# HLLMR/stratum-dsp

Measured on AMD Instinct MI355X. Metric: tracks/sec full analyze_audio(), 3-min 44.1 kHz mono, at 1/2/4/8 MI355X, higher is better.
Workload: dtype f32

## Files before the change

### stratum-dsp_amd/csrc/k_features.hip

```cpp
#include <stdexcept>
#include <type_traits>

#include "kernels.hpp"

namespace sdsp {



typedef const __attribute__((address_space(4))) int* ConstI;
typedef const __attribute__((address_space(4))) MelChunk* ConstMC;

template <int CW, int W, int KK>
__global__ __launch_bounds__(FT_FRAMES) __attribute__((amdgpu_waves_per_eu(KK > 0 ? 3 : 1))) void k_features(const RowMap rm,
                                                        const uint64_t* __restrict__ frame_pfx,
                                                        const uint64_t* __restrict__ tile_pfx, int T, FeatParams P,
                                                        const MelPlan* __restrict__ mel, float* __restrict__ E,
                                                        float* __restrict__ H, float* __restrict__ SFX,
                                                        float* __restrict__ SFO, float* __restrict__ MEL,
                                                        uint64_t total) {
    static_assert((W & (W - 1)) == 0, "W must be a power of two");
    constexpr int ROWS = FT_FRAMES;
    constexpr int LS = W + 1;
    __shared__ float2 ML[ROWS][LS];
    __shared__ sd_logtab2_t ltab[512];
    __shared__ sd_ln2tab_t etab[129];
    static_assert(KK == 0 || CW + 2 * KK <= W, "window halo must fit the ring");
    for (int q = threadIdx.x; q < 512; q += FT_FRAMES) ltab[q] = SD_LOGTAB9_D[q];
    for (int q = threadIdx.x; q < 129; q += FT_FRAMES) etab[q] = sd_ln2tab_from(q);

    const uint64_t gb = blockIdx.x;
    const int trk = find_track(tile_pfx, T, gb);
    const int64_t F = (int64_t)(frame_pfx[trk + 1] - frame_pfx[trk]);
    const int64_t f0 = (int64_t)(gb - tile_pfx[trk]) * FT_STEP;
    const uint64_t g0 = frame_pfx[trk];
    const int i = threadIdx.x;
    const bool helper = (i & 63) == 0;
    const int ro = i;
    const int64_t f = f0 - 1 + 63 * (i >> 6) + (i & 63);
    const bool own_ok = f >= 0 && f < F;
    const bool valid = !helper && f < F;
    const bool has_prev = valid && f >= 1;
    const int K = KK > 0 ? KK : P.K, B = P.B;
    const uint64_t g = g0 + (uint64_t)f;

    float e[4] = {0, 0, 0, 0}, h[4] = {0, 0, 0, 0}, sx[4] = {0, 0, 0, 0}, so = 0.0f;
    float eb = 0.0f, hb = 0.0f, sb = 0.0f;
    int cur = 0;
    auto band_of = [&](int b) {
        int v = 0;
#pragma unroll
        for (int q = 3; q >= 1; q--)
            if (P.band_on[q] && b >= P.bs[q] && b < P.be[q]) v = q;
        return v;
    };
    auto flush = [&]() {
        if (cur == 1) e[1] = eb, h[1] = hb, sx[1] = sb;
        else if (cur == 2) e[2] = eb, h[2] = hb, sx[2] = sb;
        else if (cur == 3) e[3] = eb, h[3] = hb, sx[3] = sb;
        eb = hb = sb = 0.0f;
    };
    float accA = 0.0f, accB = 0.0f;
    int mA = 0;
    float* melA = MEL;
    const uint32_t mel_vo = valid ? (uint32_t)g * 4u : 0xFFFFFFF0u;
    auto mel_rsrc = [&]() {
        return __builtin_amdgcn_make_buffer_rsrc((void*)melA, (short)0, (int)(uint32_t)(total * 4u), 0x00020000);
    };
    const uint64_t ra0 = rm.rowA0[trk], rb0 = rm.rowB0 ? rm.rowB0[trk] : ra0 + (uint64_t)rm.offB;
    auto row_of = [&](int64_t fr, bool* odd) {
        *odd = fr & 1;
        return (*odd ? rb0 + (uint64_t)(fr >> 1) * (uint64_t)rm.stepB : ra0 + (uint64_t)(fr >> 1) * (uint64_t)rm.stepA);
    };
    auto fmax_of = [&](int64_t fr) {
        bool odd;
        const uint64_t r = row_of(fr, &odd);
        return odd ? rm.fmaxB[r] : rm.fmaxA[r];
    };
    const float mx_c = own_ok ? fmax_of(f) : 0.0f;
    const bool cn = mx_c > EPS;
    const float yr = cn ? 1.0f / mx_c : 0.0f;
    const bool q_frame_ok = !cn || mx_c <= 0x1p100f;
    const uint32_t q_lim = __float_as_uint(sd_maxf(0x1p-100f, mx_c * 0x1p-120f)) - 1u;
    uint32_t q_lo = 0xFFFFFFFFu, q_hi = 0u;
    auto quot = [&](float m) {
        const uint32_t u = __float_as_uint(m);
        q_lo = min(q_lo, u - 1u);
        q_hi = max(q_hi, u);
        const float q0 = m * yr;
        return __builtin_fmaf(__builtin_fmaf(-mx_c, q0, m), yr, q0);
    };
    auto quot_redo = [&](int c0, int nb, float so_start) {
        const bool miss = !q_frame_ok || q_lo < q_lim || q_hi >= 0x7F800000u;
        q_lo = 0xFFFFFFFFu;
        q_hi = 0u;
        if (__builtin_expect(__builtin_amdgcn_ballot_w64(miss) == 0, 1)) return;
        so = so_start;
        for (int j = 0; j < nb; j++) {
            const float m = ML[ro][(c0 + j) & (W - 1)].x;
            const float cv = cn ? m / mx_c : 0.0f;
            const float pv = __builtin_bit_cast(
                float, __builtin_amdgcn_update_dpp(0, __builtin_bit_cast(int, cv), 0x138, 0xf, 0xf, true));
            const float d = max_bnn(cv - pv, 0.0f);
            so += d * d;
        }
    };

    const int lane = i & 63, wrow = i & ~63;
    const int sub = lane / CW, jj = lane % CW;
    const int64_t fw = f0 - 1 + 63 * (i >> 6);

    constexpr int RSTEP = 64 / CW;
    constexpr int NLD = CW;
    const float* rowp[NLD];
#pragma unroll
    for (int u = 0; u < NLD; u++) {
        const int64_t fr = fw + sub + u * RSTEP;
        rowp[u] = rm.magsA;
        if (fr >= 0 && fr < F) {
            bool odd;
            const uint64_t row = row_of(fr, &odd);
            rowp[u] = (odd ? rm.magsB : rm.magsA) + row * (uint64_t)P.stride;
        }
    }
    float nx[NLD];
    uint32_t row_ok = 0;
#pragma unroll
    for (int u = 0; u < NLD; u++) {
        const int64_t fr = fw + sub + u * RSTEP;
        row_ok |= (uint32_t)(fr >= 0 && fr < F) << u;
    }
    auto load = [&](int b0) {
        const int b = b0 + jj;
// ... 32 lines not shown
        asm volatile("" ::: "memory");
        if (c0 + CW < B) load(c0 + CW + K);
        const int nb = B - c0 < CW ? B - c0 : CW;
        if (__builtin_amdgcn_ballot_w64(valid) == 0) continue;
        float Rw[KK > 0 ? CW + 2 * KK : 1];
        constexpr bool VHK = KK > 0 && 2 * KK == CW;
        float Wm[VHK ? CW : 1];
        const int rp = lane > 0 ? ro - 1 : ro;
        if (KK > 0) {
#pragma unroll
            for (int q = 0; q < (KK > 0 ? CW + 2 * KK : 1); q++) Rw[q] = ML[rp][(c0 - KK + q) & (W - 1)].y;
            if constexpr (VHK) {
                float suf[CW], pre[CW];
                suf[CW - 1] = Rw[CW - 1];
#pragma unroll
                for (int q = CW - 2; q >= 0; q--) suf[q] = max_bnn(Rw[q], suf[q + 1]);
                pre[0] = Rw[CW];
#pragma unroll
                for (int q = 1; q < CW; q++) pre[q] = max_bnn(pre[q - 1], Rw[CW + q]);
#pragma unroll
                for (int q = 0; q < CW; q++) Wm[q] = max_bnn(suf[q], pre[q]);
            }
        }
        if constexpr (VHK) {
            const int cf = ((ConstI)P.chunk_flags)[c0 / CW];
            if (cf & (FT_CHUNK_FAST | FT_CHUNK_MEL)) {
                const int vbc = cf & 3;
                if (vbc != cur) {
                    flush();
                    cur = vbc;
                }
                const float so_start = so;
                auto walk = [&](auto mel_tag, auto reg_tag, auto noband_tag) {
                    constexpr bool MEL = decltype(mel_tag)::value;
                    constexpr bool REG = decltype(reg_tag)::value;
                    constexpr bool NOBAND = decltype(noband_tag)::value;
                    MelChunk mc{};
                    const ConstMC mcp = (ConstMC)P.mel_chunks + c0 / CW;
                    if constexpr (MEL) {
                        mc.bits = mcp->bits;
#pragma unroll
                        for (int j = 0; j < CW; j++) mc.w0[j] = mcp->w0[j], mc.w1[j] = mcp->w1[j];
                    }
                    float bfv[CW];
#pragma unroll
                    for (int j = 0; j < CW; j++) bfv[j] = mcp->bf[j];
#pragma unroll
                    for (int j = 0; j < CW; j++) {
                        const int b = c0 + j;
                        const int s = b & (W - 1);
                        const float2 ml = ML[ro][s];
                        const float m = ml.x;
                        const float ee = m * m;
                        const float hh = bfv[j] * m * m;
                        e[0] += ee;
                        h[0] += hh;
                        const float lc = ml.y;
                        const float cv = quot(m);
                        const float pv = __builtin_bit_cast(
                            float, __builtin_amdgcn_update_dpp(0, __builtin_bit_cast(int, cv), 0x138, 0xf, 0xf, true));
                        const float d = max_bnn(cv - pv, 0.0f);
                        so += d * d;
                        const float df = max_bnn(lc - Wm[j], 0.0f);
                        const float df2 = df * df;
                        sx[0] += df2;
                        if (!NOBAND && vbc) {
                            eb += ee;
                            hb += hh;
                            sb += df2;
                        }
                        if constexpr (MEL) {
                            const uint32_t pb = mc.bits >> (4 * j);
                            for (uint32_t q = pb & 3; q > 0; q--) {
                                __builtin_amdgcn_raw_buffer_store_b32(__float_as_uint(accA), mel_rsrc(), mel_vo, 0, 0);
                                accA = accB;
                                accB = 0.0f;
                                mA++;
                                melA += total;
                            }
                            if constexpr (REG) {
                                if (__float_as_uint(mc.w0[j]) << 1) accA += lc * mc.w0[j];
                                if (__float_as_uint(mc.w1[j]) << 1) accB += lc * mc.w1[j];
                            } else if (mc.w0[j] != 0.0f) {
                                if (pb & 4) accB += lc * mc.w0[j];
                                else accA += lc * mc.w0[j];
                            }
                            if (!REG && mc.w1[j] != 0.0f) {
                                if (pb & 8) accB += lc * mc.w1[j];
                                else accA += lc * mc.w1[j];
                            }
                        }
                    }
                };
                if (cf & FT_CHUNK_MELREG)
                    walk(std::true_type{}, std::true_type{}, std::false_type{});
                else if (cf & FT_CHUNK_MEL)
                    walk(std::true_type{}, std::false_type{}, std::false_type{});
                else if (vbc == 0)
                    walk(std::false_type{}, std::false_type{}, std::true_type{});
                else
                    walk(std::false_type{}, std::false_type{}, std::false_type{});
                quot_redo(c0, CW, so_start);
                continue;
            }
        }
        const float so_start = so;
#pragma unroll
        for (int j = 0; j < CW; j++) {
            if (j >= nb) continue;
            const int b = c0 + j;
            const int s = b & (W - 1);
            const float2 ml = ML[ro][s];
            const float m = ml.x;
            const float ee = m * m;
            const float hh = (float)b * m * m;
            e[0] += ee;
            h[0] += hh;
            const int vb = band_of(b);
            if (vb != cur) {
                flush();
                cur = vb;
            }
            if (vb) {
                eb += ee;
                hb += hh;
            }
            const float lc = ml.y;
            const float cv = quot(m);
            const float pv = __builtin_bit_cast(
                float, __builtin_amdgcn_update_dpp(0, __builtin_bit_cast(int, cv), 0x138 , 0xf, 0xf, true));
            if (P.n_mels > 0) {
                const MelPlan mp = mel[b];
                for (int q = 0; q < mp.nflush; q++) {
                    if (valid) MEL[(uint64_t)mA * total + g] = accA;
                    accA = accB;
                    accB = 0.0f;
                    mA++;
                    melA += total;
                }
                if (mp.w0 != 0.0f) {
                    if (mp.s0 == 0) accA += lc * mp.w0;
                    else accB += lc * mp.w0;
                }
                if (mp.w1 != 0.0f) {
                    if (mp.s1 == 0) accA += lc * mp.w1;
                    else accB += lc * mp.w1;
                }
            }
            {
                const float d = max_bnn(cv - pv, 0.0f);
                so += d * d;
                const int lo = b - K < 0 ? 0 : b - K;
                const int hi = b + K + 1 < B ? b + K + 1 : B;
                float pm = 0.0f;
                if constexpr (KK > 0) {
                    if constexpr (VHK) {
                        pm = Wm[j];
                    } else {
                        pm = Rw[j];
#pragma unroll
                        for (int q = 1; q <= 2 * KK; q++) pm = max_bnn(pm, Rw[j + q]);
                    }
                } else {
                    for (int q = lo; q < hi; q++) pm = max_bnn(pm, ML[rp][q & (W - 1)].y);
                }
                const float df = max_bnn(lc - pm, 0.0f);
                const float df2 = df * df;
                sx[0] += df2;
                if (vb) {
                    const int bsv = P.bs[vb], bev = P.be[vb];
                    if (lo < bsv || hi > bev) {
                        const int lb = lo < bsv ? bsv : lo;
                        const int hbd = hi > bev ? bev : hi;
                        float pmb = 0.0f;
                        if constexpr (KK > 0) {
#pragma unroll
                            for (int q = 0; q <= 2 * KK; q++)
                                if (b - KK + q >= lb && b - KK + q < hbd) pmb = max_bnn(pmb, Rw[j + q]);
                        } else {
                            for (int q = lb; q < hbd; q++) pmb = max_bnn(pmb, ML[rp][q & (W - 1)].y);
                        }
                        const float db = max_bnn(lc - pmb, 0.0f);
                        sb += db * db;
                    } else {
                        sb += df2;
                    }
                }
            }
        }
        quot_redo(c0, nb, so_start);
    }
    flush();
    if (!valid) return;
    for (; mA < P.n_mels; mA++) {
        MEL[(uint64_t)mA * total + g] = accA;
        accA = accB;
        accB = 0.0f;
    }
#pragma unroll
    for (int v = 0; v < 4; v++) {
        E[(uint64_t)v * total + g] = e[v];
        H[(uint64_t)v * total + g] = h[v];
    }
    if (has_prev) {
        const uint64_t gp = g - 1;
        SFO[gp] = __builtin_sqrtf(so);
#pragma unroll
        for (int v = 0; v < 4; v++) SFX[(uint64_t)v * total + gp] = __builtin_sqrtf(sx[v]);
    }
}

void launch_features(const RowMap& mags, const uint64_t* frame_pfx, const uint64_t* tile_pfx,
                     int T, uint64_t n_tiles, const FeatParams& P, const MelPlan* mel, float* E, float* H, float* SFX,
                     float* SFO, float* MEL, uint64_t total, hipStream_t st) {
    if (n_tiles == 0) return;
    if (total >= (1ull << 30)) throw std::runtime_error("launch_features: too many frames for one launch");

    if (P.K == 4)
        hipLaunchKernelGGL((k_features<8, 16, 4>), dim3((unsigned)n_tiles), dim3(FT_FRAMES), 0, st, mags,
                           frame_pfx, tile_pfx, T, P, mel, E, H, SFX, SFO, MEL, total);
    else if (P.K <= 4)
        hipLaunchKernelGGL((k_features<8, 16, 0>), dim3((unsigned)n_tiles), dim3(FT_FRAMES), 0, st, mags,
                           frame_pfx, tile_pfx, T, P, mel, E, H, SFX, SFO, MEL, total);
    else
        hipLaunchKernelGGL((k_features<16, 32, 0>), dim3((unsigned)n_tiles), dim3(FT_FRAMES), 0, st, mags,
                           frame_pfx, tile_pfx, T, P, mel, E, H, SFX, SFO, MEL, total);
}

}
```

### stratum-dsp_amd/csrc/kernels.hpp

```cpp
#pragma once

#include <hip/hip_runtime.h>
#include <stdint.h>

#include "sdsp_device.hpp"

namespace sdsp {

constexpr int NVAR = 5;

struct MelChunk {
    uint32_t bits;
    float w0[8], w1[8];
    float bf[8];
};
struct FeatParams {
    int B;
    int stride;
    int K;
    int bs[4], be[4];
    int band_on[4];
    int n_mels;
    const int* chunk_flags;
    const MelChunk* mel_chunks;
};
constexpr int FT_CHUNK_FAST = 4, FT_CHUNK_MEL = 8, FT_CHUNK_MELREG = 16;
struct MelPlan {
    int nflush;
    int s0, s1;
    float w0, w1;
};
#ifndef SDSP_PK_CH
#define SDSP_PK_CH 16384
#endif
constexpr int PK_CH = SDSP_PK_CH;
constexpr int FT_FRAMES = 256;
constexpr int FT_STEP = FT_FRAMES - FT_FRAMES / 64;
struct RowMap {
    const float *magsA, *magsB, *fmaxA, *fmaxB;
    const uint64_t *rowA0, *rowB0;
    int offB, stepA, stepB;
};
constexpr int FT_KMAX = 8;
constexpr int FT_MELMAX = 48;

struct NovParams {
    float ws, we, wh, wsum;
    int lmw, smw;
    int band_on[4];
};

struct FftTgParams {
    int P;
    int b_lo, K;
    float fres;
    int lds;
};
struct SelParams {
    float min_bpm, max_bpm, ac_tol;
    float w[NVAR];
// ... 176 lines not shown
void launch_loudness_gain(const float* x, const uint64_t* in_off, const uint64_t* n_raw, const uint64_t* chunk_pfx,
                          int T, uint64_t n_chunks, unsigned int* chunk_bits, unsigned int* peak_bits,
                          const LoudnessParams& P, float* gain, int* status, hipStream_t st);
void launch_frame_rms(const float* x, const uint64_t* src_off, const float* gain, const uint64_t* n_len,
                      const uint64_t* frame_pfx, int T, uint64_t total, int fs, int hop, float* rms, hipStream_t st, bool per_frame_kernel = false);
void launch_trim(const float* rms, const uint64_t* frame_pfx, int T, const uint64_t* n_raw, int hop, float thr,
                 uint64_t min_frames, int enable, uint64_t* trim_start, uint64_t* trim_end, hipStream_t st,
                 const uint64_t* base_pfx = nullptr, int stride = 1);
void launch_frame_rms_from_raw(const float* raw, const uint64_t* raw_base, const float* x, const uint64_t* src_off,
                               const float* gain, const uint64_t* n_trim, const uint64_t* frame_pfx, int T, uint64_t total,
                               int fs, int hop, float* rms, hipStream_t st);
void launch_energy_onsets(const float* rms, const uint64_t* frame_pfx, const uint64_t* n_trim, int hop, float factor,
                          uint32_t* out, const uint64_t* out_off, int* out_n, int T, hipStream_t st);
void launch_flux_onsets(const float* sfo, const float* hfc, const float* hpe, float* scratch, const uint64_t* frame_pfx,
                        const uint64_t* n_trim, int hop, float pct, uint32_t* out, const uint64_t* out_off,
                        int* out_n, int T, hipStream_t st);
void launch_consensus(const uint32_t* energy, const uint64_t* e_off, const int* e_n, const uint32_t* flux_on,
                      const uint64_t* f_off, const int* f_n, uint64_t kind_stride, int T, uint32_t tol, int enable,
                      const int* has_mags, uint32_t* chosen, const uint64_t* c_off, int* c_n, uint32_t* scratch,
                      hipStream_t st, int hpss = 0);
void launch_features(const RowMap& mags, const uint64_t* frame_pfx, const uint64_t* tile_pfx,
                     int T, uint64_t n_tiles, const FeatParams& P, const MelPlan* mel, float* E, float* H, float* SFX,
                     float* SFO, float* MEL, uint64_t total, hipStream_t st);
void launch_novelty(const float* E, const float* H, const float* SFX, const uint64_t* frame_pfx, int T, uint64_t total,
                    const NovParams& P, float* scratch, float* nov, float* nov_sum, const float* MEL, int n_mels,
                    int mel_k, bool mel_on, unsigned int* mel_max, hipStream_t st);
void launch_fft_tempogram(const int* items, int n_items, int T, const float* nov, const float* nov_sum,
                          const uint64_t* frame_pfx, uint64_t total, const FftTgParams& P, const cx* tw, const cx* rt,
                          cx* gscratch, const uint64_t* out_off, float* out_bpm, float* out_pow, hipStream_t st);
void launch_acf_tempogram(const int* items, int n_items, const float* nov, const uint64_t* frame_pfx, uint64_t total,
                          const float* bpm_grid, const int* lag_grid, int NB, float* out_bpm, float* out_str,
                          hipStream_t st);
void launch_tempo_select(int n_items, const int* active, const float* fft_bpm, const float* fft_pow, const uint64_t* fft_off,
                         const int* fft_k, const float* acf_bpm, const float* acf_str, const uint64_t* acf_off,
                         const SelParams& P, TempoEst* est, float* cand, int cand_cap, hipStream_t st);
void launch_multires(const int* tracks, int n_items, const float* c256, const int* n256, const float* c512,
                     const int* n512, const float* c1024, const int* n1024, int cap256, int cap512, int cap1024,
                     const TempoEst* base_est, const float* nov512, const uint64_t* fpfx512, const MrParams& P,
                     TempoEst* mr_est, int* used, float* final_bpm, float* final_conf, hipStream_t st, MrDbg* dbg = nullptr);
void launch_beat(const int* tracks, int n_items, const uint32_t* onsets, const uint64_t* on_off, const int* on_n,
                 uint32_t sr, const float* bpm, const float* conf, float* scratch, const uint64_t* beat_off,
                 const int* beat_cap, float* beats, float* downs, BeatOut* out, hipStream_t st);
void launch_beat_compact(int n, const BeatOut* out, const uint64_t* beat_off, const float* beats, const float* downs,
                         uint64_t* pfx, float* cb, float* cd, hipStream_t st);
void launch_mask(float* mags, int stride, int B, const uint64_t* frame_pfx, const int* tracks, int n_items, int margin,
                 float power, hipStream_t st, bool smooth_only = false);
// ... 64 lines not shown
```

### stratum-dsp_amd/csrc/pipeline.hpp

```cpp
#pragma once
#include <algorithm>
#include <chrono>
#include <cmath>
#include <cstdio>
#include <cstdlib>
#include <cstring>
#include <deque>
#include <map>
#include <memory>
#include <string>
#include <vector>

#include "../../include/sdsp_fft_spec.h"
#include "../../include/stratum_hip_debug.h"
#include "kernels.hpp"
#include "sdsp_runtime.hpp"

namespace sdsp {
namespace detail {

int base_stride(int fs);
inline uint64_t key_fft(const sdsp_config& c) {
    return c.enable_key_stft_override ? std::max<uint64_t>(c.key_stft_frame_size, 256) : c.frame_size;
}
// ... 128 lines not shown
}
inline void set_key_fields(TrackRes& r, const TrackRes& rerun) {
    r.key_mode = rerun.key_mode;
    r.key_tonic = rerun.key_tonic;
    r.key_conf = rerun.key_conf;
    r.key_clarity = rerun.key_clarity;
}

struct PassTg {
    int present[NVAR] = {0, 0, 0, 0, 0};
    int NB = 0;
    std::vector<int> items;
    std::vector<uint64_t> fft_off;
    std::vector<int> fft_k;
    std::vector<int> fft_k_track;
    float *acf_bpm = nullptr, *acf_str = nullptr;
    float *fft_bpm = nullptr, *fft_pow = nullptr;
};
struct TempoStageDbg {
    FeatParams fp{};
    PassTg tg;
};

struct TempoPassIn {
    int hop = 0;
    const float* samples = nullptr;
    std::vector<uint64_t> src_off;
    std::vector<float> gain_h;
    std::vector<uint64_t> n_trim;
    int top_n = 0, gate = 0, cand_cap = 0;
    const float* mags_in = nullptr;
    const float* fmax_in = nullptr;
    int reuse = 0;
    const float* base_mags = nullptr;
    const float* base_fmax = nullptr;
    std::vector<uint64_t> base_row0;
    bool mr_nov = false;
    TempoStageDbg* dbg = nullptr;
};
TempoPassIn subset(const TempoPassIn& base, const std::vector<int>& which);
struct TempoPassOut {
    std::vector<uint64_t> fpfx;
    uint64_t total = 0;
    float *mags = nullptr, *fmax = nullptr, *E = nullptr, *H = nullptr, *SFX = nullptr, *SFO = nullptr, *MEL = nullptr,
          *nov = nullptr, *nov_sum = nullptr, *cand = nullptr, *nov_mr = nullptr;
    uint64_t* d_fpfx = nullptr;
    TempoEst* est = nullptr;
    int* active = nullptr;
    std::vector<int> active_h;
    double stft_ms = 0, feat_ms = 0, tempo_ms = 0;
    uint64_t stft_launch = 0;
    uint64_t stft_frames = 0;
    double stft_bytes = 0;
};
struct PassPlan {
    int P_T = 0;
    std::vector<uint64_t> tpfx;
    uint64_t* d_tpfx = nullptr;
    RowMap rm{};
};
// ... 184 lines not shown
    bool hpss_on() const { return cfg_.enable_hpss_onsets && cfg_.enable_onset_consensus; }
    bool perc_on() const { return mr_on() && cfg_.enable_tempogram_percussive_fallback; }
    bool dbg_on() const { return cfg_.has_debug_track_id != 0; }
    void add_pass_times(const TempoPassOut& o);

    void loudness_prepass(const float* d_samples, const std::vector<uint64_t>& in_off,
                          const std::vector<uint64_t>& n_raw, std::vector<TrackRes>& res);
    void sub_batch(const float* d_samples, const std::vector<uint64_t>& in_off, const std::vector<uint64_t>& n_raw,
                   const std::vector<int>& idx, std::vector<TrackRes>& res);
    Front front(const float* d_samples, const std::vector<uint64_t>& in_off, const std::vector<uint64_t>& n_raw,
                const std::vector<int>& idx, std::vector<TrackRes>& res);
    TempoPassIn base_pass_in(const float* d_samples, const Front& f) const;
    Hpss hpss(const TempoPassOut& bo, const std::vector<TempoEst>& best, HostTrace& htr);
    Onsets onsets(const float* d_samples, const Front& f, const TempoPassIn& bin, const TempoPassOut& bo, const Hpss& hp);
    Beats beat_grid(const TempoPassIn& bin, const TempoPassOut& bo, const Onsets& on, const Tempo& tp);
    ResultsHost download_results(const Beats& bt, const TempoPassIn& bin, const TempoPassOut& bo);
    Overview overview(const float* d_samples, const TempoPassIn& bin, const TempoPassOut& bo, Timers& tm);
    void overview_results(const Overview& ov, const Front& f, const TempoPassIn& bin, const TempoPassOut& bo, Timers& tm);
    void fill_results(const Front& f, const TempoPassIn& bin, const std::vector<TempoEst>& best, const Tempo& tp,
                      const ResultsHost& rh, std::vector<TrackRes>& res);

    void tempo_pass(const std::string& tag, const TempoPassIn& in, TempoPassOut& out);
    PassPlan pass_stft(const std::string& tag, const TempoPassIn& in, TempoPassOut& o, Timers& tm);
    PassFeat pass_features(const std::string& tag, const PassPlan& pl, TempoPassOut& o);
    void pass_novelty(const std::string& tag, const TempoPassIn& in, const PassPlan& pl, const PassFeat& pf,
                      TempoPassOut& o);
    PassTg pass_tempograms(const std::string& tag, const TempoPassIn& in, const PassPlan& pl, const PassFeat& pf,
                           const TempoPassOut& o);
    void pass_select(const std::string& tag, const TempoPassIn& in, const PassPlan& pl, const PassTg& tg,
                     TempoPassOut& o);
    Tempo seed_tempo(const Front& f, const std::vector<TempoEst>& best, const Onsets& on, std::vector<TrackRes>& res);
    void escalate(const Front& f, const TempoPassIn& bin, const TempoPassOut& bo, const std::vector<TempoEst>& best,
                  Tempo& tp, std::vector<TrackDbg>& tdbg, std::vector<TrackRes>& res);
    void perc_fallback(const Front& f, const TempoPassIn& bin, const TempoPassOut& bo, const std::vector<TempoEst>& best,
                       const Hpss& hp, Tempo& tp, std::vector<TrackRes>& res);
    void legacy_select(const Front& f, const TempoPassIn& bin, const Onsets& on, Tempo& tp, std::vector<TrackRes>& res);

    KeyLaunch launch_key(const float* d_samples, const TempoPassIn& bin);
    KeyCond key_condition(const std::string& EP, float* mags8, const std::vector<uint64_t>& kpfx,
                          const std::vector<uint64_t>& ktile, uint64_t* d_kpfx, uint64_t* d_ktile, int* d_kid,
                          hipStream_t st2, Timers& kt);
    void key_timeline_results(const KeyTimelineOut& ktl, const std::vector<size_t>& at, const std::vector<uint64_t>& first);
    void join_key_only(KeyLaunch& kl, const Front& f, std::vector<TrackRes>& res);
    std::vector<KeyOut> join_key(const float* d_samples, const std::vector<uint64_t>& in_off,
                                 const std::vector<uint64_t>& n_raw, const Front& f, KeyLaunch& kl, HostTrace& htr,
                                 std::vector<TrackRes>& res);
    std::vector<size_t> finish_key(std::vector<TrackRes>& res, bool keep_tail = false);
// ... 18 lines not shown
```

### stratum-dsp_amd/csrc/pipeline_tempo.hip

```cpp
#include "pipeline.hpp"

namespace sdsp {

namespace detail {
TempoPassIn subset(const TempoPassIn& base, const std::vector<int>& which) {
    TempoPassIn s;
    s.hop = base.hop;
    s.samples = base.samples;
    for (int i : which) {
        s.src_off.push_back(base.src_off[(size_t)i]);
        s.gain_h.push_back(base.gain_h[(size_t)i]);
        s.n_trim.push_back(base.n_trim[(size_t)i]);
    }
    return s;
}
}

static uint64_t next_pow2(uint64_t n) {
    uint64_t p = 1;
    while (p < n) p <<= 1;
    return p;
}

void Pipeline::add_pass_times(const TempoPassOut& o) {
    times_.stft2048_ms += o.stft_ms;
    times_.stft2048_launches += o.stft_launch;
    times_.stft2048_frames += o.stft_frames;
    times_.stft2048_bytes += o.stft_bytes;
    times_.features_ms += o.feat_ms;
    times_.tempogram_ms += o.tempo_ms;
}

void Pipeline::tempo_pass(const std::string& tag, const TempoPassIn& in, TempoPassOut& o) {
    Timers tm;
    tm.init(d_);
    const PassPlan pl = pass_stft(tag, in, o, tm);
    tm.mark(1);
    const PassFeat pf = pass_features(tag, pl, o);
    pass_novelty(tag, in, pl, pf, o);
    tm.mark(2);
    const PassTg tg = pass_tempograms(tag, in, pl, pf, o);
    pass_select(tag, in, pl, tg, o);
    tm.mark(3);
    if (in.dbg) {
        in.dbg->fp = pf.fp;
        in.dbg->tg = tg;
    }
    c_.sync();
    o.stft_ms = tm.ms(0, 1);
    o.feat_ms = tm.ms(1, 2);
    o.tempo_ms = tm.ms(2, 3);
}

PassPlan Pipeline::pass_stft(const std::string& tag, const TempoPassIn& in, TempoPassOut& o, Timers& tm) {
    PassPlan pl;
    const int P_T = pl.P_T = (int)in.src_off.size();
    const int FS = fs_, hop = in.hop;
    o.fpfx.assign((size_t)P_T + 1, 0);
    pl.tpfx.assign((size_t)P_T + 1, 0);
    o.active_h.assign((size_t)P_T, 0);
    for (int t = 0; t < P_T; t++) {
        const uint64_t n = in.n_trim[(size_t)t];
        const uint64_t F = n >= (uint64_t)FS ? (n - FS) / (uint64_t)hop + 1 : 0;
        o.fpfx[(size_t)t + 1] = o.fpfx[(size_t)t] + F;
        pl.tpfx[(size_t)t + 1] = pl.tpfx[(size_t)t] + (F + FT_STEP - 1) / FT_STEP;
        o.active_h[(size_t)t] = F >= 2;
    }
    const uint64_t total = o.total = o.fpfx[(size_t)P_T];
    o.d_fpfx = c_.up(tag + "fpfx", o.fpfx);
    pl.d_tpfx = c_.up(tag + "tpfx", pl.tpfx);
    uint64_t* d_src = c_.up(tag + "src", in.src_off);
    float* d_gain = c_.up(tag + "gain", in.gain_h);
    o.active = c_.up(tag + "active", o.active_h);
    FftTables& tb = d_.tables(FS, true);
    tm.mark(0);
    uint64_t stft_frames = 0;
    if (in.mags_in) {
        o.mags = const_cast<float*>(in.mags_in);
        o.fmax = const_cast<float*>(in.fmax_in);
    } else if (in.reuse == 1) {
        o.mags = nullptr;
        o.fmax = nullptr;
        pl.rm = RowMap{in.base_mags, in.base_mags, in.base_fmax, in.base_fmax, c_.up(tag + "brow", in.base_row0), nullptr,
                       2, 4, 4};
    } else if (in.reuse == 2) {
        std::vector<uint64_t> opfx((size_t)P_T + 1, 0), osrc((size_t)P_T);
        for (int t = 0; t < P_T; t++) {
            opfx[(size_t)t + 1] = opfx[(size_t)t] + (o.fpfx[(size_t)t + 1] - o.fpfx[(size_t)t]) / 2;
            osrc[(size_t)t] = in.src_off[(size_t)t] + (uint64_t)hop;
        }
        stft_frames = opfx[(size_t)P_T];
        o.mags = c_.dev<float>(tag + "mags", std::max<uint64_t>(stft_frames, 1) * s2_);
        o.fmax = c_.dev<float>(tag + "fmax", std::max<uint64_t>(stft_frames, 1));
        uint64_t* d_opfx = c_.up(tag + "opfx", opfx);
        const std::vector<uint64_t> ostr = stft_strips(opfx);
        launch_stft(FS, true, in.samples, d_opfx, P_T, stft_frames, c_.up(tag + "osrc", osrc), d_gain, 2 * hop,
                    tb.window.as<float>(), stft_twp(tb, FS, true), stft_rtp(tb, FS, true), o.mags, d_opfx, s2_, o.fmax,
                    d_.stream, c_.up(tag + "ostrip", ostr), ostr.back(), c_.dev<uint32_t>(tag + "redo", stft_frames + 1));
        SDSP_HIP_CHECK(hipGetLastError());
        pl.rm = RowMap{in.base_mags, o.mags, in.base_fmax, o.fmax, c_.up(tag + "brow", in.base_row0), d_opfx, 0, 1, 1};
    } else {
        o.mags = c_.dev<float>(tag + "mags", total * s2_);
        o.fmax = c_.dev<float>(tag + "fmax", total);
        const std::vector<uint64_t> str = stft_strips(o.fpfx);
        launch_stft(FS, true, in.samples, o.d_fpfx, P_T, total, d_src, d_gain, hop, tb.window.as<float>(),
                    stft_twp(tb, FS, true), stft_rtp(tb, FS, true), o.mags, o.d_fpfx, s2_, o.fmax, d_.stream,
                    c_.up(tag + "strip", str), str.back(), c_.dev<uint32_t>(tag + "redo", total + 1));
        SDSP_HIP_CHECK(hipGetLastError());
        stft_frames = total;
    }
    if (in.mags_in || in.reuse == 0) pl.rm = RowMap{o.mags, o.mags, o.fmax, o.fmax, o.d_fpfx, nullptr, 1, 2, 2};
    o.stft_launch = stft_frames ? 1 : 0;
    o.stft_frames = stft_frames;
    if (stft_frames) {
        double inb = 0;
        for (int t = 0; t < P_T; t++) inb += 4.0 * (double)in.n_trim[(size_t)t];
        o.stft_bytes = inb + 4.0 * (double)stft_frames * (double)nb_;
    }
    return pl;
}

PassFeat Pipeline::pass_features(const std::string& tag, const PassPlan& pl, TempoPassOut& o) {
    PassFeat pf;
    const int B = nb_;
    const uint64_t total = o.total;
    pf.configured = band_configured(cfg_);
    pf.mel_on = pf.configured && cfg_.enable_tempogram_mel_novelty;
    FeatParams& fp = pf.fp = feat_params(cfg_, sr_, B, s2_);
    std::string merr;
    MelTable mt = mel_table(sr_, B, (int)cfg_.tempogram_mel_n_mels, cfg_.tempogram_mel_fmin_hz, cfg_.tempogram_mel_fmax_hz,
                            &merr);
    if (!merr.empty()) throw HipError(merr);
    std::vector<MelPlan> mplan = mel_plan(mt, B, &merr);
    if (!merr.empty()) throw HipError(merr);
    MelPlan* d_mplan = c_.up(tag + "melplan", mplan);
    std::vector<int> cf;
    std::vector<MelChunk> mc;
    feat_chunk_tables(fp, mplan, &cf, &mc);
    fp.chunk_flags = c_.up(tag + "ftchunk", cf);
    fp.mel_chunks = c_.up(tag + "ftmelchunk", mc);
    o.E = c_.dev<float>(tag + "E", 4 * total);
    o.H = c_.dev<float>(tag + "H", 4 * total);
    o.SFX = c_.dev<float>(tag + "SFX", 4 * total);
    o.SFO = c_.dev<float>(tag + "SFO", total);
    o.MEL = c_.dev<float>(tag + "MEL", std::max<uint64_t>(total * (uint64_t)std::max(fp.n_mels, 1), 1));
    launch_features(pl.rm, o.d_fpfx, pl.d_tpfx, pl.P_T, pl.tpfx[(size_t)pl.P_T], fp, d_mplan, o.E, o.H, o.SFX, o.SFO,
                    o.MEL, total, d_.stream);
    SDSP_HIP_CHECK(hipGetLastError());
    return pf;
}

void Pipeline::pass_novelty(const std::string& tag, const TempoPassIn& in, const PassPlan& pl, const PassFeat& pf,
                            TempoPassOut& o) {
    const int P_T = pl.P_T;
    const uint64_t total = o.total;
    NovParams np = nov_params(cfg_, pf.configured);
    for (int v = 0; v < 4; v++) np.band_on[v] = pf.fp.band_on[v];
    float* scratch = c_.dev<float>(tag + "novscr", 8 * std::max<uint64_t>(total, 1));
    o.nov = c_.dev<float>(tag + "nov", NVAR * std::max<uint64_t>(total, 1));
    o.nov_sum = c_.dev<float>(tag + "novsum", NVAR * (size_t)std::max(P_T, 1));
    launch_novelty(o.E, o.H, o.SFX, o.d_fpfx, P_T, total, np, scratch, o.nov, o.nov_sum, o.MEL, pf.fp.n_mels,
                   (int)std::max<uint64_t>(cfg_.tempogram_mel_max_filter_bins, 1), pf.mel_on,
                   c_.dev<unsigned int>(tag + "melmax", (size_t)std::max(P_T, 1)), d_.stream);
    SDSP_HIP_CHECK(hipGetLastError());
    o.nov_mr = o.nov;
    if (in.mr_nov && !pf.configured) {
        NovParams nm = nov_params(cfg_, true);
        nm.band_on[0] = np.band_on[0];
// ... 136 lines not shown
    tp.d_used = c_.up("B.used", tp.used);
    if (mr_on() && !E.empty()) {
        const int NE = (int)E.size();
        const int top_k = (int)std::max<uint64_t>(cfg_.tempogram_multi_res_top_k, 1);
        const int aux_k = std::min(std::max(top_k * 4, 25), 200);
        TempoPassIn ein = subset(bin, E);
        const bool own512 = bin.hop != 512;
        TempoPassOut o256, o512, o1024;
        if (own512) {
            ein.hop = 512;
            ein.top_n = top_k;
            ein.cand_cap = top_k;
            ein.mr_nov = true;
            tempo_pass("C512.", ein, o512);
            ein.mr_nov = false;
        }
        const TempoPassOut& b512 = own512 ? o512 : bo;
        ein.base_mags = b512.mags;
        ein.base_fmax = b512.fmax;
        for (int k = 0; k < NE; k++) ein.base_row0.push_back(b512.fpfx[own512 ? (size_t)k : (size_t)E[(size_t)k]]);
        ein.top_n = aux_k;
        ein.cand_cap = aux_k;
        const bool reuse_on = test_hooks().no_row_reuse.load() == 0;
        ein.hop = 256;
        ein.reuse = reuse_on ? 2 : 0;
        tempo_pass("C256.", ein, o256);
        ein.hop = 1024;
        ein.reuse = reuse_on ? 1 : 0;
        tempo_pass("C1024.", ein, o1024);
        add_pass_times(o256);
        add_pass_times(o1024);
        if (own512) add_pass_times(o512);
        std::vector<TempoEst> e256 = c_.down(o256.est, (size_t)NE), e1024 = c_.down(o1024.est, (size_t)NE);
        std::vector<int> n256((size_t)NE), n1024((size_t)NE), n512((size_t)NR);
        for (int k = 0; k < NE; k++) {
            n256[(size_t)k] = e256[(size_t)k].ok ? e256[(size_t)k].n_cands : -1;
            n1024[(size_t)k] = e1024[(size_t)k].ok ? e1024[(size_t)k].n_cands : -1;
        }
        if (own512) {
            const std::vector<TempoEst> e512 = c_.down(o512.est, (size_t)NE);
            n512.assign((size_t)NE, 0);
            for (int k = 0; k < NE; k++)
                n512[(size_t)k] = e512[(size_t)k].ok ? std::min(e512[(size_t)k].n_cands, top_k) : -1;
            if (cfg_.emit_tempogram_candidates) {
                tp.c512_h = c_.down(o512.cand, (size_t)NE * (size_t)top_k * 4);
                tp.n512_own = n512;
                tp.c512_cap = top_k;
            }
        } else {
            for (int i = 0; i < NR; i++) n512[(size_t)i] = std::min(best[(size_t)i].n_cands, top_k);
        }
// ... 155 lines not shown
```

Before: 3044.

## Fuse hop-1024 SuperFlux into hop-256 feature pass and gather other features from hop-512

The hop-256 feature kernel gains a variant that skips the unused spectral-flux (SFO) work and also computes the hop-1024 SuperFlux, using a 4-frame lag window built with ds_bpermute. The hop-1024 pass then takes SFX from that fused output and copies E/H/MEL from the hop-512 pass through a strided gather kernel instead of rerunning the full feature kernel. The hop-256 STFT also skips computing fmax when flux is not needed. This removes one full feature-kernel pass per track, at the cost of more helper lanes per tile (4 instead of 1), extra registers in the hop-256 kernel, and more complex cross-pass dependencies.

```diff
diff --git a/stratum-dsp_amd/csrc/k_features.hip b/stratum-dsp_amd/csrc/k_features.hip
--- a/stratum-dsp_amd/csrc/k_features.hip
+++ b/stratum-dsp_amd/csrc/k_features.hip
@@ -10,15 +10,23 @@
 typedef const __attribute__((address_space(4))) int* ConstI;
 typedef const __attribute__((address_space(4))) MelChunk* ConstMC;
 
-template <int CW, int W, int KK>
-__global__ __launch_bounds__(FT_FRAMES) __attribute__((amdgpu_waves_per_eu(KK > 0 ? 3 : 1))) void k_features(const RowMap rm,
-                                                        const uint64_t* __restrict__ frame_pfx,
-                                                        const uint64_t* __restrict__ tile_pfx, int T, FeatParams P,
-                                                        const MelPlan* __restrict__ mel, float* __restrict__ E,
-                                                        float* __restrict__ H, float* __restrict__ SFX,
-                                                        float* __restrict__ SFO, float* __restrict__ MEL,
-                                                        uint64_t total) {
+struct FeatX4 {
+    const uint64_t* frame_pfx4;
+    float* SFX4;
+    uint64_t total4;
+};
+
+template <int CW, int W, int KK, bool FLUX, bool X4>
+__device__ __forceinline__ void features_body(const RowMap rm, const uint64_t* __restrict__ frame_pfx,
+                                              const uint64_t* __restrict__ tile_pfx, int T, FeatParams P,
+                                              const MelPlan* __restrict__ mel, float* __restrict__ E,
+                                              float* __restrict__ H, float* __restrict__ SFX,
+                                              float* __restrict__ SFO, float* __restrict__ MEL, uint64_t total,
+                                              const FeatX4 x4) {
     static_assert((W & (W - 1)) == 0, "W must be a power of two");
+    static_assert(!X4 || (KK > 0 && 2 * KK == CW), "the fused hop-1024 SuperFlux is built for the split window maxima");
+    constexpr int HR = X4 ? 4 : 1;
+    constexpr int WF = 64 - HR;
     constexpr int ROWS = FT_FRAMES;
     constexpr int LS = W + 1;
     __shared__ float2 ML[ROWS][LS];
@@ -31,12 +39,12 @@
     const uint64_t gb = blockIdx.x;
     const int trk = find_track(tile_pfx, T, gb);
     const int64_t F = (int64_t)(frame_pfx[trk + 1] - frame_pfx[trk]);
-    const int64_t f0 = (int64_t)(gb - tile_pfx[trk]) * FT_STEP;
+    const int64_t f0 = (int64_t)(gb - tile_pfx[trk]) * (X4 ? FT_STEP_X4 : FT_STEP);
     const uint64_t g0 = frame_pfx[trk];
     const int i = threadIdx.x;
-    const bool helper = (i & 63) == 0;
+    const bool helper = (i & 63) < HR;
     const int ro = i;
-    const int64_t f = f0 - 1 + 63 * (i >> 6) + (i & 63);
+    const int64_t f = f0 - HR + WF * (i >> 6) + (i & 63);
     const bool own_ok = f >= 0 && f < F;
     const bool valid = !helper && f < F;
     const bool has_prev = valid && f >= 1;
@@ -45,6 +53,7 @@
 
     float e[4] = {0, 0, 0, 0}, h[4] = {0, 0, 0, 0}, sx[4] = {0, 0, 0, 0}, so = 0.0f;
     float eb = 0.0f, hb = 0.0f, sb = 0.0f;
+    float sx4[4] = {0, 0, 0, 0}, sb4 = 0.0f;
     int cur = 0;
     auto band_of = [&](int b) {
         int v = 0;
@@ -54,10 +63,10 @@
         return v;
     };
     auto flush = [&]() {
-        if (cur == 1) e[1] = eb, h[1] = hb, sx[1] = sb;
-        else if (cur == 2) e[2] = eb, h[2] = hb, sx[2] = sb;
-        else if (cur == 3) e[3] = eb, h[3] = hb, sx[3] = sb;
-        eb = hb = sb = 0.0f;
+        if (cur == 1) e[1] = eb, h[1] = hb, sx[1] = sb, sx4[1] = sb4;
+        else if (cur == 2) e[2] = eb, h[2] = hb, sx[2] = sb, sx4[2] = sb4;
+        else if (cur == 3) e[3] = eb, h[3] = hb, sx[3] = sb, sx4[3] = sb4;
+        eb = hb = sb = sb4 = 0.0f;
     };
     float accA = 0.0f, accB = 0.0f;
     int mA = 0;
@@ -76,7 +85,7 @@
         const uint64_t r = row_of(fr, &odd);
         return odd ? rm.fmaxB[r] : rm.fmaxA[r];
     };
-    const float mx_c = own_ok ? fmax_of(f) : 0.0f;
+    const float mx_c = FLUX && own_ok ? fmax_of(f) : 0.0f;
     const bool cn = mx_c > EPS;
     const float yr = cn ? 1.0f / mx_c : 0.0f;
     const bool q_frame_ok = !cn || mx_c <= 0x1p100f;
@@ -107,7 +116,7 @@
 
     const int lane = i & 63, wrow = i & ~63;
     const int sub = lane / CW, jj = lane % CW;
-    const int64_t fw = f0 - 1 + 63 * (i >> 6);
+    const int64_t fw = f0 - HR + WF * (i >> 6);
 
     constexpr int RSTEP = 64 / CW;
     constexpr int NLD = CW;
@@ -186,6 +195,14 @@
                 for (int q = 0; q < CW; q++) Wm[q] = max_bnn(suf[q], pre[q]);
             }
         }
+        const int rp4 = lane >= 4 ? ro - 4 : ro;
+        float Wm4[X4 ? CW : 1];
+        if constexpr (X4) {
+            const int src = ((lane - 3) & 63) * 4;
+#pragma unroll
+            for (int q = 0; q < CW; q++)
+                Wm4[q] = __builtin_bit_cast(float, __builtin_amdgcn_ds_bpermute(src, __builtin_bit_cast(int, Wm[q])));
+        }
         if constexpr (VHK) {
             const int cf = ((ConstI)P.chunk_flags)[c0 / CW];
             if (cf & (FT_CHUNK_FAST | FT_CHUNK_MEL)) {
@@ -220,11 +237,13 @@
                         e[0] += ee;
                         h[0] += hh;
                         const float lc = ml.y;
-                        const float cv = quot(m);
-                        const float pv = __builtin_bit_cast(
-                            float, __builtin_amdgcn_update_dpp(0, __builtin_bit_cast(int, cv), 0x138, 0xf, 0xf, true));
-                        const float d = max_bnn(cv - pv, 0.0f);
-                        so += d * d;
+                        if constexpr (FLUX) {
+                            const float cv = quot(m);
+                            const float pv = __builtin_bit_cast(
+                                float, __builtin_amdgcn_update_dpp(0, __builtin_bit_cast(int, cv), 0x138, 0xf, 0xf, true));
+                            const float d = max_bnn(cv - pv, 0.0f);
+                            so += d * d;
+                        }
                         const float df = max_bnn(lc - Wm[j], 0.0f);
                         const float df2 = df * df;
                         sx[0] += df2;
@@ -232,6 +251,12 @@
                             eb += ee;
                             hb += hh;
                             sb += df2;
+                        }
+                        if constexpr (X4) {
+                            const float d4 = max_bnn(lc - Wm4[j], 0.0f);
+                            const float d42 = d4 * d4;
+                            sx4[0] += d42;
+                            if (!NOBAND && vbc) sb4 += d42;
                         }
                         if constexpr (MEL) {
                             const uint32_t pb = mc.bits >> (4 * j);
@@ -264,7 +289,7 @@
                     walk(std::false_type{}, std::false_type{}, std::true_type{});
                 else
                     walk(std::false_type{}, std::false_type{}, std::false_type{});
-                quot_redo(c0, CW, so_start);
+                if constexpr (FLUX) quot_redo(c0, CW, so_start);
                 continue;
             }
         }
@@ -290,7 +315,7 @@
                 hb += hh;
             }
             const float lc = ml.y;
-            const float cv = quot(m);
+            const float cv = FLUX ? quot(m) : 0.0f;
             const float pv = __builtin_bit_cast(
                 float, __builtin_amdgcn_update_dpp(0, __builtin_bit_cast(int, cv), 0x138 , 0xf, 0xf, true));
             if (P.n_mels > 0) {
@@ -312,8 +337,10 @@
                 }
             }
             {
-                const float d = max_bnn(cv - pv, 0.0f);
-                so += d * d;
+                if constexpr (FLUX) {
+                    const float d = max_bnn(cv - pv, 0.0f);
+                    so += d * d;
+                }
                 const int lo = b - K < 0 ? 0 : b - K;
                 const int hi = b + K + 1 < B ? b + K + 1 : B;
                 float pm = 0.0f;
@@ -350,9 +377,30 @@
                         sb += df2;
                     }
                 }
+                if constexpr (X4) {
+                    const float d4 = max_bnn(lc - Wm4[j], 0.0f);
+                    const float d42 = d4 * d4;
+                    sx4[0] += d42;
+                    if (vb) {
+                        const int bsv = P.bs[vb], bev = P.be[vb];
+                        if (lo < bsv || hi > bev) {
+                            const int lb = lo < bsv ? bsv : lo;
+                            const int hbd = hi > bev ? bev : hi;
+                            float pmb = 0.0f;
+#pragma unroll
+                            for (int q = 0; q <= 2 * KK; q++)
+                                if (b - KK + q >= lb && b - KK + q < hbd)
+                                    pmb = max_bnn(pmb, ML[rp4][(b - KK + q) & (W - 1)].y);
+                            const float db = max_bnn(lc - pmb, 0.0f);
+                            sb4 += db * db;
+                        } else {
+                            sb4 += d42;
+                        }
+                    }
+                }
             }
         }
-        quot_redo(c0, nb, so_start);
+        if constexpr (FLUX) quot_redo(c0, nb, so_start);
     }
     flush();
     if (!valid) return;
@@ -368,10 +416,58 @@
     }
     if (has_prev) {
         const uint64_t gp = g - 1;
-        SFO[gp] = __builtin_sqrtf(so);
+        if constexpr (FLUX) SFO[gp] = __builtin_sqrtf(so);
 #pragma unroll
         for (int v = 0; v < 4; v++) SFX[(uint64_t)v * total + gp] = __builtin_sqrtf(sx[v]);
     }
+    if constexpr (X4) {
+        if (f >= 4 && (f & 3) == 0) {
+            const uint64_t g4 = x4.frame_pfx4[trk] + (uint64_t)(f >> 2) - 1;
+#pragma unroll
+            for (int v = 0; v < 4; v++) x4.SFX4[(uint64_t)v * x4.total4 + g4] = __builtin_sqrtf(sx4[v]);
+        }
+    }
+}
+
+template <int CW, int W, int KK>
+__global__ __launch_bounds__(FT_FRAMES) __attribute__((amdgpu_waves_per_eu(KK > 0 ? 3 : 1))) void k_features(const RowMap rm,
+                                                        const uint64_t* __restrict__ frame_pfx,
+                                                        const uint64_t* __restrict__ tile_pfx, int T, FeatParams P,
+                                                        const MelPlan* __restrict__ mel, float* __restrict__ E,
+                                                        float* __restrict__ H, float* __restrict__ SFX,
+                                                        float* __restrict__ SFO, float* __restrict__ MEL,
+                                                        uint64_t total) {
+    features_body<CW, W, KK, true, false>(rm, frame_pfx, tile_pfx, T, P, mel, E, H, SFX, SFO, MEL, total, FeatX4{});
+}
+
+template <bool X4>
+__global__ __launch_bounds__(FT_FRAMES) __attribute__((amdgpu_waves_per_eu(3))) void k_features_esc(
+    const RowMap rm, const uint64_t* __restrict__ frame_pfx, const uint64_t* __restrict__ tile_pfx, int T, FeatParams P,
+    const MelPlan* __restrict__ mel, float* __restrict__ E, float* __restrict__ H, float* __restrict__ SFX,
+    float* __restrict__ MEL, uint64_t total, FeatX4 x4) {
+    features_body<8, 16, 4, false, X4>(rm, frame_pfx, tile_pfx, T, P, mel, E, H, SFX, nullptr, MEL, total, x4);
+}
+
+__global__ __launch_bounds__(256) void k_features_gather2(const uint64_t* __restrict__ frame_pfx4,
+                                                          const uint64_t* __restrict__ row0, int T,
+                                                          const uint64_t* __restrict__ tile_pfx,
+                                                          const float* __restrict__ E2, const float* __restrict__ H2,
+                                                          const float* __restrict__ MEL2, uint64_t total2,
+                                                          float* __restrict__ E4, float* __restrict__ H4,
+                                                          float* __restrict__ MEL4, uint64_t total4) {
+    const uint64_t gb = blockIdx.x;
+    const int trk = find_track(tile_pfx, T, gb);
+    const uint64_t F = frame_pfx4[trk + 1] - frame_pfx4[trk];
+    const uint64_t j = (gb - tile_pfx[trk]) * 256u + threadIdx.x;
+    if (j >= F) return;
+    const uint64_t src = row0[trk] + 2 * j, dst = frame_pfx4[trk] + j;
+    const int r = blockIdx.y;
+    if (r < 4)
+        E4[(uint64_t)r * total4 + dst] = E2[(uint64_t)r * total2 + src];
+    else if (r < 8)
+        H4[(uint64_t)(r - 4) * total4 + dst] = H2[(uint64_t)(r - 4) * total2 + src];
+    else
+        MEL4[(uint64_t)(r - 8) * total4 + dst] = MEL2[(uint64_t)(r - 8) * total2 + src];
 }
 
 void launch_features(const RowMap& mags, const uint64_t* frame_pfx, const uint64_t* tile_pfx,
@@ -391,4 +487,28 @@
                            frame_pfx, tile_pfx, T, P, mel, E, H, SFX, SFO, MEL, total);
 }
 
-}
+
+void launch_features_esc(const RowMap& mags, const uint64_t* frame_pfx, const uint64_t* tile_pfx, int T, uint64_t n_tiles,
+                         const FeatParams& P, const MelPlan* mel, float* E, float* H, float* SFX, float* MEL, uint64_t total,
+                         const uint64_t* frame_pfx4, float* SFX4, uint64_t total4, hipStream_t st) {
+    if (n_tiles == 0) return;
+    if (total >= (1ull << 30)) throw std::runtime_error("launch_features_esc: too many frames for one launch");
+    if (P.K != 4) throw std::runtime_error("launch_features_esc: built for a SuperFlux half width of 4");
+    const FeatX4 x4{frame_pfx4, SFX4, total4};
+    if (SFX4)
+        hipLaunchKernelGGL(k_features_esc<true>, dim3((unsigned)n_tiles), dim3(FT_FRAMES), 0, st, mags, frame_pfx,
+                           tile_pfx, T, P, mel, E, H, SFX, MEL, total, x4);
+    else
+        hipLaunchKernelGGL(k_features_esc<false>, dim3((unsigned)n_tiles), dim3(FT_FRAMES), 0, st, mags, frame_pfx,
+                           tile_pfx, T, P, mel, E, H, SFX, MEL, total, x4);
+}
+
+void launch_features_gather2(const uint64_t* frame_pfx4, const uint64_t* row0, int T, const uint64_t* tile_pfx,
+                             uint64_t n_tiles, int n_mels, const float* E2, const float* H2, const float* MEL2,
+                             uint64_t total2, float* E4, float* H4, float* MEL4, uint64_t total4, hipStream_t st) {
+    if (n_tiles == 0) return;
+    hipLaunchKernelGGL(k_features_gather2, dim3((unsigned)n_tiles, (unsigned)(8 + n_mels)), dim3(256), 0, st, frame_pfx4,
+                       row0, T, tile_pfx, E2, H2, MEL2, total2, E4, H4, MEL4, total4);
+}
+
+}
diff --git a/stratum-dsp_amd/csrc/kernels.hpp b/stratum-dsp_amd/csrc/kernels.hpp
--- a/stratum-dsp_amd/csrc/kernels.hpp
+++ b/stratum-dsp_amd/csrc/kernels.hpp
@@ -36,6 +36,7 @@
 constexpr int PK_CH = SDSP_PK_CH;
 constexpr int FT_FRAMES = 256;
 constexpr int FT_STEP = FT_FRAMES - FT_FRAMES / 64;
+constexpr int FT_STEP_X4 = FT_FRAMES - 4 * (FT_FRAMES / 64);
 struct RowMap {
     const float *magsA, *magsB, *fmaxA, *fmaxB;
     const uint64_t *rowA0, *rowB0;
@@ -258,6 +259,12 @@
 void launch_features(const RowMap& mags, const uint64_t* frame_pfx, const uint64_t* tile_pfx,
                      int T, uint64_t n_tiles, const FeatParams& P, const MelPlan* mel, float* E, float* H, float* SFX,
                      float* SFO, float* MEL, uint64_t total, hipStream_t st);
+void launch_features_esc(const RowMap& mags, const uint64_t* frame_pfx, const uint64_t* tile_pfx, int T, uint64_t n_tiles,
+                         const FeatParams& P, const MelPlan* mel, float* E, float* H, float* SFX, float* MEL, uint64_t total,
+                         const uint64_t* frame_pfx4, float* SFX4, uint64_t total4, hipStream_t st);
+void launch_features_gather2(const uint64_t* frame_pfx4, const uint64_t* row0, int T, const uint64_t* tile_pfx,
+                             uint64_t n_tiles, int n_mels, const float* E2, const float* H2, const float* MEL2,
+                             uint64_t total2, float* E4, float* H4, float* MEL4, uint64_t total4, hipStream_t st);
 void launch_novelty(const float* E, const float* H, const float* SFX, const uint64_t* frame_pfx, int T, uint64_t total,
                     const NovParams& P, float* scratch, float* nov, float* nov_sum, const float* MEL, int n_mels,
                     int mel_k, bool mel_on, unsigned int* mel_max, hipStream_t st);
diff --git a/stratum-dsp_amd/csrc/pipeline.hpp b/stratum-dsp_amd/csrc/pipeline.hpp
--- a/stratum-dsp_amd/csrc/pipeline.hpp
+++ b/stratum-dsp_amd/csrc/pipeline.hpp
@@ -174,6 +174,7 @@
     PassTg tg;
 };
 
+struct TempoPassOut;
 struct TempoPassIn {
     int hop = 0;
     const float* samples = nullptr;
@@ -188,6 +189,12 @@
     const float* base_fmax = nullptr;
     std::vector<uint64_t> base_row0;
     bool mr_nov = false;
+    bool no_flux = false;
+    float* sfx4_out = nullptr;
+    const uint64_t* sfx4_fpfx = nullptr;
+    uint64_t sfx4_total = 0;
+    float* sfx_in = nullptr;
+    const TempoPassOut* feat512 = nullptr;
     TempoStageDbg* dbg = nullptr;
 };
 TempoPassIn subset(const TempoPassIn& base, const std::vector<int>& which);
@@ -418,7 +425,7 @@
 
     void tempo_pass(const std::string& tag, const TempoPassIn& in, TempoPassOut& out);
     PassPlan pass_stft(const std::string& tag, const TempoPassIn& in, TempoPassOut& o, Timers& tm);
-    PassFeat pass_features(const std::string& tag, const PassPlan& pl, TempoPassOut& o);
+    PassFeat pass_features(const std::string& tag, const TempoPassIn& in, const PassPlan& pl, TempoPassOut& o);
     void pass_novelty(const std::string& tag, const TempoPassIn& in, const PassPlan& pl, const PassFeat& pf,
                       TempoPassOut& o);
     PassTg pass_tempograms(const std::string& tag, const TempoPassIn& in, const PassPlan& pl, const PassFeat& pf,
diff --git a/stratum-dsp_amd/csrc/pipeline_tempo.hip b/stratum-dsp_amd/csrc/pipeline_tempo.hip
--- a/stratum-dsp_amd/csrc/pipeline_tempo.hip
+++ b/stratum-dsp_amd/csrc/pipeline_tempo.hip
@@ -36,7 +36,7 @@
     tm.init(d_);
     const PassPlan pl = pass_stft(tag, in, o, tm);
     tm.mark(1);
-    const PassFeat pf = pass_features(tag, pl, o);
+    const PassFeat pf = pass_features(tag, in, pl, o);
     pass_novelty(tag, in, pl, pf, o);
     tm.mark(2);
     const PassTg tg = pass_tempograms(tag, in, pl, pf, o);
@@ -56,6 +56,7 @@
     PassPlan pl;
     const int P_T = pl.P_T = (int)in.src_off.size();
     const int FS = fs_, hop = in.hop;
+    const uint64_t tstep = in.sfx_in ? 256 : in.sfx4_out ? FT_STEP_X4 : FT_STEP;
     o.fpfx.assign((size_t)P_T + 1, 0);
     pl.tpfx.assign((size_t)P_T + 1, 0);
     o.active_h.assign((size_t)P_T, 0);
@@ -63,7 +64,7 @@
         const uint64_t n = in.n_trim[(size_t)t];
         const uint64_t F = n >= (uint64_t)FS ? (n - FS) / (uint64_t)hop + 1 : 0;
         o.fpfx[(size_t)t + 1] = o.fpfx[(size_t)t] + F;
-        pl.tpfx[(size_t)t + 1] = pl.tpfx[(size_t)t] + (F + FT_STEP - 1) / FT_STEP;
+        pl.tpfx[(size_t)t + 1] = pl.tpfx[(size_t)t] + (F + tstep - 1) / tstep;
         o.active_h[(size_t)t] = F >= 2;
     }
     const uint64_t total = o.total = o.fpfx[(size_t)P_T];
@@ -91,11 +92,12 @@
         }
         stft_frames = opfx[(size_t)P_T];
         o.mags = c_.dev<float>(tag + "mags", std::max<uint64_t>(stft_frames, 1) * s2_);
-        o.fmax = c_.dev<float>(tag + "fmax", std::max<uint64_t>(stft_frames, 1));
+        const bool fm = !in.no_flux || stft_general(FS, true) != stft_general(FS, false);
+        o.fmax = fm ? c_.dev<float>(tag + "fmax", std::max<uint64_t>(stft_frames, 1)) : nullptr;
         uint64_t* d_opfx = c_.up(tag + "opfx", opfx);
         const std::vector<uint64_t> ostr = stft_strips(opfx);
-        launch_stft(FS, true, in.samples, d_opfx, P_T, stft_frames, c_.up(tag + "osrc", osrc), d_gain, 2 * hop,
-                    tb.window.as<float>(), stft_twp(tb, FS, true), stft_rtp(tb, FS, true), o.mags, d_opfx, s2_, o.fmax,
+        launch_stft(FS, fm, in.samples, d_opfx, P_T, stft_frames, c_.up(tag + "osrc", osrc), d_gain, 2 * hop,
+                    tb.window.as<float>(), stft_twp(tb, FS, fm), stft_rtp(tb, FS, fm), o.mags, d_opfx, s2_, o.fmax,
                     d_.stream, c_.up(tag + "ostrip", ostr), ostr.back(), c_.dev<uint32_t>(tag + "redo", stft_frames + 1));
         SDSP_HIP_CHECK(hipGetLastError());
         pl.rm = RowMap{in.base_mags, o.mags, in.base_fmax, o.fmax, c_.up(tag + "brow", in.base_row0), d_opfx, 0, 1, 1};
@@ -120,13 +122,24 @@
     return pl;
 }
 
-PassFeat Pipeline::pass_features(const std::string& tag, const PassPlan& pl, TempoPassOut& o) {
+PassFeat Pipeline::pass_features(const std::string& tag, const TempoPassIn& in, const PassPlan& pl, TempoPassOut& o) {
     PassFeat pf;
     const int B = nb_;
     const uint64_t total = o.total;
     pf.configured = band_configured(cfg_);
     pf.mel_on = pf.configured && cfg_.enable_tempogram_mel_novelty;
     FeatParams& fp = pf.fp = feat_params(cfg_, sr_, B, s2_);
+    if (in.sfx_in) {
+        const TempoPassOut& b = *in.feat512;
+        o.E = c_.dev<float>(tag + "E", 4 * total);
+        o.H = c_.dev<float>(tag + "H", 4 * total);
+        o.SFX = in.sfx_in;
+        o.MEL = c_.dev<float>(tag + "MEL", std::max<uint64_t>(total * (uint64_t)std::max(fp.n_mels, 1), 1));
+        launch_features_gather2(o.d_fpfx, pl.rm.rowA0, pl.P_T, pl.d_tpfx, pl.tpfx[(size_t)pl.P_T], fp.n_mels, b.E, b.H, b.MEL,
+                                b.total, o.E, o.H, o.MEL, total, d_.stream);
+        SDSP_HIP_CHECK(hipGetLastError());
+        return pf;
+    }
     std::string merr;
     MelTable mt = mel_table(sr_, B, (int)cfg_.tempogram_mel_n_mels, cfg_.tempogram_mel_fmin_hz, cfg_.tempogram_mel_fmax_hz,
                             &merr);
@@ -142,8 +155,14 @@
     o.E = c_.dev<float>(tag + "E", 4 * total);
     o.H = c_.dev<float>(tag + "H", 4 * total);
     o.SFX = c_.dev<float>(tag + "SFX", 4 * total);
+    o.MEL = c_.dev<float>(tag + "MEL", std::max<uint64_t>(total * (uint64_t)std::max(fp.n_mels, 1), 1));
+    if (in.no_flux) {
+        launch_features_esc(pl.rm, o.d_fpfx, pl.d_tpfx, pl.P_T, pl.tpfx[(size_t)pl.P_T], fp, d_mplan, o.E, o.H, o.SFX, o.MEL,
+                            total, in.sfx4_fpfx, in.sfx4_out, in.sfx4_total, d_.stream);
+        SDSP_HIP_CHECK(hipGetLastError());
+        return pf;
+    }
     o.SFO = c_.dev<float>(tag + "SFO", total);
-    o.MEL = c_.dev<float>(tag + "MEL", std::max<uint64_t>(total * (uint64_t)std::max(fp.n_mels, 1), 1));
     launch_features(pl.rm, o.d_fpfx, pl.d_tpfx, pl.P_T, pl.tpfx[(size_t)pl.P_T], fp, d_mplan, o.E, o.H, o.SFX, o.SFO,
                     o.MEL, total, d_.stream);
     SDSP_HIP_CHECK(hipGetLastError());
@@ -326,11 +345,28 @@
         ein.top_n = aux_k;
         ein.cand_cap = aux_k;
         const bool reuse_on = test_hooks().no_row_reuse.load() == 0;
+        const bool fused = reuse_on && !dbg_on() && feat_params(cfg_, sr_, nb_, s2_).K == 4;
         ein.hop = 256;
         ein.reuse = reuse_on ? 2 : 0;
+        if (fused) {
+            std::vector<uint64_t> fpfx4((size_t)NE + 1, 0);
+            for (int k = 0; k < NE; k++) {
+                const uint64_t n = ein.n_trim[(size_t)k];
+                fpfx4[(size_t)k + 1] = fpfx4[(size_t)k] + (n >= (uint64_t)fs_ ? (n - (uint64_t)fs_) / 1024 + 1 : 0);
+            }
+            ein.no_flux = true;
+            ein.sfx4_total = fpfx4[(size_t)NE];
+            ein.sfx4_fpfx = c_.up("C256.fpfx4", fpfx4);
+            ein.sfx4_out = c_.dev<float>("C1024.SFX", 4 * ein.sfx4_total);
+        }
         tempo_pass("C256.", ein, o256);
         ein.hop = 1024;
         ein.reuse = reuse_on ? 1 : 0;
+        if (fused) {
+            ein.sfx_in = ein.sfx4_out;
+            ein.sfx4_out = nullptr;
+            ein.feat512 = &b512;
+        }
         tempo_pass("C1024.", ein, o1024);
         add_pass_times(o256);
         add_pass_times(o1024);
```

Result: faster. 3113, median of 6 (+2.3%).
